# BBillot/SynthSR

Measured on AMD Instinct MI355X. Metric: training volumes/sec (160^3 fp32, 5-level U-Net), higher is better.
Workload: dtype f32; 1 GPU; configs[1]: brain_generator 160^3 batch=1 (training() defaults) + 5-level 3-D U-Net (24..384 features, Cin=2) fwd/bwd + Adam, fp32, random-init; global_batch=1, parallelism=dp1, conv_arithmetic=split

## Files before the change

synthsr_amd/csrc/conv3d.hip:

```cpp
#include "common.h"
#include <algorithm>
#include <cstddef>

SYN_DET_SETTER(conv3d)

namespace {

typedef float f32x4 __attribute__((ext_vector_type(4)));

constexpr int MAX_NT = 6;

__host__ __device__ inline int cdiv(int a, int b) { return (a + b - 1) / b; }

inline int ck_for(int Cin) { return (Cin % 24 == 0) ? 24 : 8; }
inline int ck_for_fwd(int Cin) { return (Cin % 24 == 0) ? 24 : ((Cin % 32 == 0) ? 32 : 8); }

template <int I, int N, class F>
__device__ __forceinline__ void sfor(F&& f) {
  if constexpr (I < N) {
    f(std::integral_constant<int, I>{});
    sfor<I + 1, N>(f);
  }
}
typedef unsigned int u32x4 __attribute__((ext_vector_type(4)));
// ... 54 lines not shown
      for (int c = 0; c < nx; ++c) v += w[((int64_t)((tz[a] * 3 + ty[b]) * 3 + tx[c]) * Cin_total + ci) * Cout + co];
  return v;
}

__host__ __device__ inline int64_t split_plane_floats(int NT, int ncc, int nchunks) {
  const int MT = NT <= -300 ? -300 - NT : (NT <= -200 ? -200 - NT : -100 - NT);
  return (int64_t)nchunks * ncc * (NT <= -200 ? 2 : 7) * MT * 64 * 4;
}
__device__ __forceinline__ void split_pack_pair(const float* __restrict__ w, int64_t i, int Cin_total, int ci_off, int Cin, int Cout,
                                                int mode, int ncc, int NT, int parity, int nchunks, uint32_t pc[3]) {
  const bool up = NT <= -200, fwdwin = NT <= -300;
  const int MT = fwdwin ? -300 - NT : (up ? -200 - NT : -100 - NT), nstep = up ? 2 : 7;
  uint32_t r = (uint32_t)i * 2u;
  const int j = (int)(r & 7);
  r >>= 3;
  const int lane = (int)(r & 63);
  r >>= 6;
  const int mt = (int)(r % MT);
  r /= MT;
  const int step = (int)(r % nstep);
  r /= nstep;
  const int cc = (int)(r % ncc);
  const int chunk = (int)(r / ncc);
  (void)nchunks;
  const int coe = (chunk * MT + mt) * 16 + (lane & 15);
  int tap;
  if (up) {
    const int t8 = syn_split_tap8(4 * step + (lane >> 4));
    const int pz = (parity >> 2) & 1, py = (parity >> 1) & 1, px = parity & 1;
    const int hz = (fwdwin ? pz : 1 - pz) + (t8 >> 2), hy = (fwdwin ? py : 1 - py) + ((t8 >> 1) & 1),
              hx = (fwdwin ? px : 1 - px) + (t8 & 1);
    tap = (hz * 3 + hy) * 3 + hx;
  } else {
    tap = syn_split_tap(4 * step + (lane >> 4));
  }
  float v0 = 0.f, v1 = 0.f;
  if (tap >= 0) {
    v0 = weight_value(w, tap, cc * 8 + j, coe, Cin_total, ci_off, Cin, Cout, mode, parity);
    v1 = weight_value(w, tap, cc * 8 + j + 1, coe, Cin_total, ci_off, Cin, Cout, mode, parity);
  }
  syn_split3(v0, v1, pc[0], pc[1], pc[2]);
}

__device__ __forceinline__ float stacked_pack_value(const float* __restrict__ w, int64_t idx, int Cin_total, int ci_off, int Cin,
                                                    int Cout, int mode) {
  uint32_t r = (uint32_t)idx * 2u;
  const int j = (int)(r & 7);
  r >>= 3;
  const int lane = (int)(r & 63);
  r >>= 6;
  const int tile = (int)(r % 5);
  r /= 5;
  const int step = (int)(r % 7);
  const int cc = (int)(r / 7);
  const int m = lane & 15;
  const int tap = syn_split_tap(4 * step + (lane >> 4));
  int piece, co;
  if (tile < 3) { piece = tile; co = m; }
  else if (tile == 3) { piece = m < 8 ? 0 : 1; co = 16 + (m & 7); }
  else { piece = m < 8 ? 2 : -1; co = 16 + (m & 7); }
  if (tap < 0 || piece < 0) return 0.f;
  const float v0 = weight_value(w, tap, cc * 8 + j, co, Cin_total, ci_off, Cin, Cout, mode, -1);
  const float v1 = weight_value(w, tap, cc * 8 + j + 1, co, Cin_total, ci_off, Cin, Cout, mode, -1);
  uint32_t pc[3];
  syn_split3(v0, v1, pc[0], pc[1], pc[2]);
  return __uint_as_float(pc[piece]);
}

__device__ __forceinline__ float pack_value(const float* __restrict__ w, int64_t idx, int Cin_total, int ci_off, int Cin,
                                            int Cout, int mode, int CK, int ncc, int NT, int parity, int NV,
                                            int64_t mfma_count) {
  if (NT == -400) return stacked_pack_value(w, idx, Cin_total, ci_off, Cin, Cout, mode);
  if (NT <= -100) {
    const int64_t n3 = split_plane_floats(NT, ncc, (int)mfma_count);
    uint32_t pc[3];
    split_pack_pair(w, idx % n3, Cin_total, ci_off, Cin, Cout, mode, ncc, NT, parity, (int)mfma_count, pc);
    return __uint_as_float(pc[idx / n3]);
  }
  if (NT < 0) {
    const int cin = -NT;
    const int lane = (int)(idx & 63);
    const int G = (int)(idx >> 6) * 16 + (lane >> 2);
    const int k = G / 6, g = G % 6;
    if (k >= 27 * cin) return 0.f;
    return weight_value(w, k / cin, k % cin, g * 4 + (lane & 3), Cin_total, ci_off, Cin, Cout, mode, parity);
  }
  if (NT == 0) {
    const int lane = (int)(idx & 63);
    uint32_t r = (uint32_t)(idx >> 6);
    const int rr = (int)(r % 3);
    r /= 3;
    const int qp = (int)(r % 3);
    r /= 3;
    const int tap = (int)(r % 27);
    const int cc = (int)(r / 27);
    const int G = rr * 16 + (lane >> 2);
    const int cie = cc * 24 + qp * 8 + (G / 24) * 4 + (G % 24) / 6;
    const int coe = (G % 6) * 4 + (lane & 3);
    return weight_value(w, tap, cie, coe, Cin_total, ci_off, Cin, Cout, mode, parity);
  }
  if (idx >= mfma_count) {
    uint32_t r = (uint32_t)(idx - mfma_count);
    const int v = (int)(r % NV);
    r /= NV;
    const int cil = (int)(r % CK);
    r /= CK;
    const int tap = (int)(r % 27);
    const int cc = (int)(r / 27);
    const int coutE = mode ? Cin : Cout;
    return weight_value(w, tap, cc * CK + cil, coutE - NV + v, Cin_total, ci_off, Cin, Cout, mode, parity);
  }
  const int NCG = CK / 8;
  uint32_t r = (uint32_t)idx;
  const int s = (int)(r & 1);
  r >>= 1;
  const int lane = (int)(r & 63);
  r >>= 6;
  const int nt = (int)(r % NT);
  r /= NT;
  const int cg = (int)(r % NCG);
  r /= NCG;
  const int tap = (int)(r % 27);
  r /= 27;
  const int cc = (int)(r % ncc);
  const int nc = (int)(r / ncc);
  const int kq = lane >> 4, j = lane & 15;
  const int cie = cc * CK + cg * 8 + 2 * kq + s;
  const int coe = (nc * NT + nt) * 16 + j;
  const int coutE = mode ? Cin : Cout;
  if (coe >= coutE - NV) return 0.f;
  return weight_value(w, tap, cie, coe, Cin_total, ci_off, Cin, Cout, mode, parity);
}

__global__ void pack_kernel(const float* __restrict__ w, float* __restrict__ packed, int Cin_total, int ci_off, int Cin,
                            int Cout, int mode, int CK, int ncc, int NT, int nchunks, int parity, int NV,
                            int64_t mfma_count, int64_t total) {
  if (NT <= -100 && NT != -400) {
    const int64_t n3 = total / 3;
    for (int64_t i = blockIdx.x * (int64_t)blockDim.x + threadIdx.x; i < n3; i += (int64_t)gridDim.x * blockDim.x) {
      uint32_t pc[3];
      split_pack_pair(w, i, Cin_total, ci_off, Cin, Cout, mode, ncc, NT, parity, (int)mfma_count, pc);
      packed[i] = __uint_as_float(pc[0]);
      packed[i + n3] = __uint_as_float(pc[1]);
      packed[i + 2 * n3] = __uint_as_float(pc[2]);
    }
    return;
  }
  for (int64_t idx = blockIdx.x * (int64_t)blockDim.x + threadIdx.x; idx < total;
       idx += (int64_t)gridDim.x * blockDim.x)
    packed[idx] = pack_value(w, idx, Cin_total, ci_off, Cin, Cout, mode, CK, ncc, NT, parity, NV, mfma_count);
}

constexpr int PACK_JOB_FIELDS = 14;
__global__ void pack_all_kernel(const float* __restrict__ params, float* __restrict__ packed,
                                const int64_t* __restrict__ jobs) {
  const int64_t* jb = jobs + (int64_t)blockIdx.y * PACK_JOB_FIELDS;
  const float* w = params + jb[0];
  float* dst = packed + jb[1];
  const int64_t count = jb[2];
  const int cin_total = (int)jb[3], ci_off = (int)jb[4], cin = (int)jb[5], cout = (int)jb[6], mode = (int)jb[7],
            ck = (int)jb[8], ncc = (int)jb[9], nt = (int)jb[10], parity = (int)jb[11], nv = (int)jb[12];
  const int64_t mfma_count = jb[13];
  if (nt <= -100 && nt != -400) {
    const int64_t n3 = count / 3;
    for (int64_t i = blockIdx.x * (int64_t)blockDim.x + threadIdx.x; i < n3; i += (int64_t)gridDim.x * blockDim.x) {
      uint32_t pc[3];
      split_pack_pair(w, i, cin_total, ci_off, cin, cout, mode, ncc, nt, parity, (int)mfma_count, pc);
      dst[i] = __uint_as_float(pc[0]);
      dst[i + n3] = __uint_as_float(pc[1]);
      dst[i + 2 * n3] = __uint_as_float(pc[2]);
    }
    return;
  }
  if (nt > 0 && parity >= 0 && parity < 8 && nv == 0) {
    const int64_t inner = (int64_t)(ck / 8) * nt * 128, count8 = count / 27 * 8;
    const int pz = (parity >> 2) & 1, py = (parity >> 1) & 1, px = parity & 1;
    for (int64_t i8 = blockIdx.x * (int64_t)blockDim.x + threadIdx.x; i8 < count8; i8 += (int64_t)gridDim.x * blockDim.x) {
      const int64_t q = i8 / inner, rem = i8 - q * inner;
      const int t8 = (int)(q & 7);
      const int slot = ((pz + (t8 >> 2)) * 3 + py + ((t8 >> 1) & 1)) * 3 + px + (t8 & 1);
      const int64_t idx = ((q >> 3) * 27 + (mode ? 26 - slot : slot)) * inner + rem;
      dst[idx] = pack_value(w, idx, cin_total, ci_off, cin, cout, mode, ck, ncc, nt, parity, nv, mfma_count);
    }
    return;
  }
  for (int64_t idx = blockIdx.x * (int64_t)blockDim.x + threadIdx.x; idx < count;
       idx += (int64_t)gridDim.x * blockDim.x)
    dst[idx] = pack_value(w, idx, cin_total, ci_off, cin, cout, mode, ck, ncc, nt, parity, nv, mfma_count);
}

__global__ void up_unpack_kernel(const float* __restrict__ dwc, float* __restrict__ dw, int Cin_total, int ci_off, int Cl,
                                 int Cout, int64_t total) {
  for (int64_t idx = blockIdx.x * (int64_t)blockDim.x + threadIdx.x; idx < total;
       idx += (int64_t)gridDim.x * blockDim.x) {
    const int co = (int)(idx % Cout);
    const int ci = (int)((idx / Cout) % Cl);
    const int t = (int)(idx / ((int64_t)Cout * Cl));
    const int tz = t / 9, ty = (t / 3) % 3, tx = t % 3;
    float acc = 0.f;
    for (int p = 0; p < 8; ++p) {
      const int pz = (p >> 2) & 1, py = (p >> 1) & 1, px = p & 1;
      const int sz = pz ? (tz == 2 ? 2 : 1) : (tz == 0 ? 0 : 1);
      const int sy = py ? (ty == 2 ? 2 : 1) : (ty == 0 ? 0 : 1);
      const int sx = px ? (tx == 2 ? 2 : 1) : (tx == 0 ? 0 : 1);
      acc += dwc[(((int64_t)p * 27 + (sz * 3 + sy) * 3 + sx) * Cl + ci) * Cout + co];
    }
    dw[((int64_t)t * Cin_total + ci_off + ci) * Cout + co] += acc;
  }
}
__global__ void up_clear_kernel(float* __restrict__ dwc, int Cl, int Cout, int64_t total64) {
  const int64_t inner = (int64_t)Cl * Cout;
  for (int64_t idx = blockIdx.x * (int64_t)blockDim.x + threadIdx.x; idx < total64; idx += (int64_t)gridDim.x * blockDim.x) {
    const int q = (int)(idx / inner);
    const int64_t rem = idx - (int64_t)q * inner;
    const int p = q >> 3, t8 = q & 7;
    const int slot = ((((p >> 2) & 1) + (t8 >> 2)) * 3 + ((p >> 1) & 1) + ((t8 >> 1) & 1)) * 3 + (p & 1) + (t8 & 1);
    dwc[((int64_t)p * 27 + slot) * inner + rem] = 0.f;
  }
}

template <int NT, int MT, bool RELU = false>
__device__ __forceinline__ void store_tile_rows(f32x4 (&acc)[MT][NT], float* slab, float* __restrict__ out,
                                                const float* __restrict__ bias, const float* addend, int act, int nc,
                                                int gz, int y0, int x0, int D1, int D2, int Cout, int lane) {
  const int li = lane & 15, kq = lane >> 4;
  constexpr int NW = NT * 16;
  const int c_lo = nc * NW;
  const int wc = min(Cout - c_lo, NW);
  const int wc4 = wc >> 2;
  const int nx = min(16, D2 - x0);
#pragma unroll
  for (int m = 0; m < MT; ++m) {
    const int gy = y0 + m;
    if (gy >= D1) continue;
#pragma unroll
    for (int n = 0; n < NT; ++n) {
      const int co = c_lo + n * 16 + li;
      const float bv = (bias && co < Cout) ? bias[co] : 0.f;
#pragma unroll
      for (int r = 0; r < 4; ++r) slab[(kq * 4 + r) * NW + n * 16 + li] = acc[m][n][r] + bv;
    }
    __builtin_amdgcn_wave_barrier();
    const size_t rowoff = (((size_t)gz * D1 + gy) * D2 + x0) * Cout + c_lo;
    for (int idx = lane; idx < nx * wc4; idx += 64) {
      const int x = idx / wc4, c4 = idx - x * wc4;
      float4 v = *reinterpret_cast<const float4*>(&slab[x * NW + c4 * 4]);
      const size_t o = rowoff + (size_t)x * Cout + c4 * 4;
      if (act == 2) {
        const float4 a = *reinterpret_cast<const float4*>(addend + o);
        v.x *= act_dy<RELU>(a.x);
        v.y *= act_dy<RELU>(a.y);
        v.z *= act_dy<RELU>(a.z);
        v.w *= act_dy<RELU>(a.w);
      } else if (addend) {
        const float4 a = *reinterpret_cast<const float4*>(addend + o);
        v.x += a.x;
        v.y += a.y;
        v.z += a.z;
        v.w += a.w;
      }
      if (act == 1) {
        v.x = act_f<RELU>(v.x);
        v.y = act_f<RELU>(v.y);
        v.z = act_f<RELU>(v.z);
        v.w = act_f<RELU>(v.w);
      }
      *reinterpret_cast<float4*>(out + o) = v;
    }
    __builtin_amdgcn_wave_barrier();
  }
}

constexpr int FT0 = 4, FT2 = 16;
constexpr int FH0 = 6, FH2 = 18;

struct ConvExt {
  int mode;
  const float* addend;
  int64_t wstride;
  int64_t valu_off;
};

__host__ __device__ inline uint32_t up_tapmask(int p, bool flipped) {
  uint32_t m = 0;
  for (int sz = 0; sz < 3; ++sz)
    for (int sy = 0; sy < 3; ++sy)
      for (int sx = 0; sx < 3; ++sx) {
        const int pz = (p >> 2) & 1, py = (p >> 1) & 1, px = p & 1;
        const bool ok = (pz ? sz >= 1 : sz <= 1) && (py ? sy >= 1 : sy <= 1) && (px ? sx >= 1 : sx <= 1);
        if (ok) {
          const int t = flipped ? (((2 - sz) * 3 + (2 - sy)) * 3 + (2 - sx)) : ((sz * 3 + sy) * 3 + sx);
          m |= 1u << t;
        }
      }
  return m;
}

template <int CK, int NT, int MT, bool KSPLIT, int NV, bool RELU = false>
__global__ __launch_bounds__(256, 2) void conv3d_fwd_kernel(const float* __restrict__ in, const float* __restrict__ wp,
                                                            const float* __restrict__ bias, float* __restrict__ out,
                                                            int D0, int D1, int D2, int Cin, int Cout, int ncc,
                                                            int tiles1, int tiles2, int act, ConvExt ext) {
  extern __shared__ __attribute__((aligned(16))) float lds[];
  constexpr int FT1 = MT, FH1 = MT + 2, FHV = FH0 * FH1 * FH2;
  constexpr int CKP = CK + 4;
  constexpr int NCG = CK / 8;
  constexpr int C4 = CK / 4;
  const int dbg = act >> 8;
  act &= 0xff;
  const int tid = threadIdx.x, lane = tid & 63, wave = tid >> 6;
  int t;
  {
    const int nwg = gridDim.x, b = blockIdx.x;
    const int q = nwg >> 3, r = nwg & 7, xcd = b & 7, j = b >> 3;
    t = (xcd < r ? xcd * (q + 1) : r * (q + 1) + (xcd - r) * q) + j;
  }
  const int t2 = t % tiles2;
  t /= tiles2;
  const int t1 = t % tiles1;
  const int t0 = t / tiles1;
  const int z0 = t0 * FT0, y0 = t1 * FT1, x0 = t2 * FT2;
  const int nc = blockIdx.y;

  f32x4 acc[MT][NT];
#pragma unroll
  for (int m = 0; m < MT; ++m)
#pragma unroll
    for (int n = 0; n < NT; ++n) acc[m][n] = (f32x4){0.f, 0.f, 0.f, 0.f};

  static_assert(NV == 0 || (MT == 4 && !KSPLIT && CK == 24), "VALU share needs the 4x4x16 tile");
  float accv[NV > 0 ? NV : 1];
#pragma unroll
  for (int v = 0; v < (NV > 0 ? NV : 1); ++v) accv[v] = 0.f;
  const int vbase = ((wave * FH1 + (lane >> 4)) * FH2 + (lane & 15)) * CKP;

  const int li = lane & 15, kq = lane >> 4;
  int a_base[MT];
#pragma unroll
  for (int m = 0; m < MT; ++m) a_base[m] = ((wave * FH1 + m) * FH2 + li) * CKP + 2 * kq;

  const float* wl = wp + (size_t)nc * ncc * 27 * NCG * NT * 128 + lane * 2;
// ... 3024 lines not shown
                       tiles2, ntiles);
  else
    hipLaunchKernelGGL(conv3d_wgrad_c2_kernel<1>, dim3(gx), dim3(256), 0, st, in, dout, partial, s[0], s[1], s[2], tiles1,
                       tiles2, ntiles);
  if (hipGetLastError() != hipSuccess) return SYNTHSR_ELAUNCH;
  const int nrow = 27 * Cin;
  hipLaunchKernelGGL(rows_reduce_kernel, dim3(cdiv((nrow + 1) * 24, 64), 32), dim3(64), 0, st, partial, gx, dw, dbias, nrow,
                     Cin, ext.cin_total, ext.ci_off);
  return hipGetLastError() == hipSuccess ? SYNTHSR_OK : SYNTHSR_ELAUNCH;
}

template <int NTAPS>
int dispatch_wgrad(const float* in, const float* dout, float* dw, const int shape[3], int Cin, int Cout, hipStream_t st,
                   const WgExt& ext) {
  if constexpr (NTAPS == 8) {
    if (up_wgrad_takes_split(shape, Cin, Cout)) {
      const int rc = syn_split_upwgrad(in, dout, dw, shape, Cin, Cout, cfg().nprod, st);
      if (rc != SYNTHSR_EINVAL) return rc;
    }
    const int64_t vox = (int64_t)shape[0] * shape[1] * shape[2];
    const int tiles0 = cdiv(shape[0], FT0), tiles1 = cdiv(shape[1], 4), tiles2 = cdiv(shape[2], FT2);
    const int ntiles = tiles0 * tiles1 * tiles2, ncc = Cin / 24;
    if (Cout == 24 && (Cin % 24) == 0 && PLAN_P4 && ntiles >= 768 && vox * Cin * 4 < (1ll << 31) &&
        vox * 8 * Cout * 4 < (1ll << 31) && !(PLAN_DBG & 16)) {
      const size_t smem = (size_t)FH0 * 6 * FH2 * 28 * sizeof(float);
      static SynOncePerDevice attr_done;
      if (auto once_ = attr_done.first()) {
        (void)hipFuncSetAttribute(reinterpret_cast<const void*>(conv3d_up_wgrad_p4_kernel),
                                  hipFuncAttributeMaxDynamicSharedMemorySize, (int)smem);
      }
      int gx = std::max(8, ((512 / (ncc * 2)) / 8) * 8);
      while (gx > 8 && gx > ntiles) gx -= 8;
      DetRun det;
      float* no_dbias = nullptr;
      if (const int rc_ = syn_det_prepare(&det, &dw, &no_dbias, 8 * ext.dwstride, Cout, gx, st)) return rc_;
      hipLaunchKernelGGL(conv3d_up_wgrad_p4_kernel, dim3(gx, ncc * 2), dim3(256), smem, st, in, dout, dw, shape[0], shape[1],
                         shape[2], Cin, tiles1, tiles2, ntiles, ext.dwstride, ext.dbg, det.stride);
      if (hipGetLastError() != hipSuccess) return SYNTHSR_ELAUNCH;
      return syn_det_finish(&det, st);
    }
  }
  if constexpr (NTAPS == 27) {
    if (Cin <= 2 && Cout == 24 && PLAN_P4 && (int64_t)shape[0] * shape[1] * shape[2] * Cout * 4 < (1ll << 31))
      return launch_wgrad_c2(in, dout, dw, ext.dbias, shape, Cin, st, ext);
    if (wgrad_takes_split(shape, Cin, Cout)) {
      const int rc = syn_split_wgrad(in, dout, dw, ext.dbias, shape, ext.cin_total, ext.ci_off, Cin, Cout, cfg().nprod, st);
      if (rc != SYNTHSR_EINVAL) return rc;
    }
  }
  if constexpr (NTAPS == 27) {
    const int64_t vox = (int64_t)shape[0] * shape[1] * shape[2];
    if (Cout == 24 && (Cin % 24) == 0 && PLAN_P4 && vox * Cin * 4 < (1ll << 31) && vox * Cout * 4 < (1ll << 31) &&
        !(PLAN_DBG & 16)) {
      const int tiles0 = cdiv(shape[0], FT0), tiles1 = cdiv(shape[1], 4), tiles2 = cdiv(shape[2], FT2);
      const int ntiles = tiles0 * tiles1 * tiles2, ncc = Cin / 24;
      const size_t smem = (size_t)FH0 * 6 * FH2 * 28 * sizeof(float);
      static SynOncePerDevice attr_done;
      if (auto once_ = attr_done.first()) {
        (void)hipFuncSetAttribute(reinterpret_cast<const void*>(conv3d_wgrad_p4_kernel),
                                  hipFuncAttributeMaxDynamicSharedMemorySize, (int)smem);
      }
      int gx = std::max(8, ((512 / ncc) / 8) * 8);
      while (gx > 8 && gx > ntiles) gx -= 8;
      DetRun det;
      float* dbias = ext.dbias;
      if (const int rc_ = syn_det_prepare(&det, &dw, &dbias, (int64_t)27 * ext.cin_total * Cout, Cout, gx, st)) return rc_;
      hipLaunchKernelGGL(conv3d_wgrad_p4_kernel, dim3(gx, ncc), dim3(256), smem, st, in, dout, dw, shape[0], shape[1],
                         shape[2], Cin, tiles1, tiles2, ntiles, ext.cin_total, ext.ci_off, ext.dbg, dbias, det.stride);
      if (hipGetLastError() != hipSuccess) return SYNTHSR_ELAUNCH;
      return syn_det_finish(&det, st);
    }
  }
  const int CK = ck_for(Cin);
  const int nt_all = cdiv(Cout, 16);
  const int nco = cdiv(nt_all, 3);
  const int NT = cdiv(nt_all, nco);
  if (CK == 24) {
    if (NT == 1) return launch_wgrad<24, 1, 1, NTAPS>(in, dout, dw, shape, Cin, Cout, st, ext);
    if (NT == 2) return launch_wgrad<24, 2, 1, NTAPS>(in, dout, dw, shape, Cin, Cout, st, ext);
    if constexpr (NTAPS == 27) return launch_wgrad<24, 3, 2, 27>(in, dout, dw, shape, Cin, Cout, st, ext);
    return launch_wgrad<24, 3, 1, NTAPS>(in, dout, dw, shape, Cin, Cout, st, ext);
  }
  if (NT == 1) return launch_wgrad<8, 1, 1, NTAPS>(in, dout, dw, shape, Cin, Cout, st, ext);
  if (NT == 2) return launch_wgrad<8, 2, 1, NTAPS>(in, dout, dw, shape, Cin, Cout, st, ext);
  return launch_wgrad<8, 3, 1, NTAPS>(in, dout, dw, shape, Cin, Cout, st, ext);
}

}

extern "C" {

int64_t synthsr_conv3d_pack_ex(const synthsr_conv_ctx* ctx, const float* w, float* packed, const int shape[3], int Cin_total,
                               int ci_off, int Cin, int Cout, int mode, int up, synthsr_stream_t stream) {
  const CtxScope scope(ctx);
  if (!scope.ok) return SYNTHSR_EINVAL;
  if (!shape || Cin < 1 || Cout < 1 || ci_off < 0 || ci_off + Cin > Cin_total || (mode != 0 && mode != 1) ||
      shape[0] < 1 || shape[1] < 1 || shape[2] < 1 || up < 0 || up > 2)
    return SYNTHSR_EINVAL;
  const int CinE = mode ? Cout : Cin, CoutE = mode ? Cin : Cout;
  const int kind = !up ? 1 : ((up == 1) == (mode == 0) ? 2 : 0);
  const FwdPlan pl = plan_fwd(shape, CinE, CoutE, kind);
  const int64_t per = pl.count();
  if (per >= (1ll << 31)) return SYNTHSR_EINVAL;
  const int64_t total = per * (up ? 8 : 1);
  if (!packed) return total;
  if (!w) return SYNTHSR_EINVAL;
  for (int p = 0; p < (up ? 8 : 1); ++p) {
    hipLaunchKernelGGL(pack_kernel, dim3(syn_grid(per, 256)), dim3(256), 0, (hipStream_t)stream, w, packed + p * per,
                       Cin_total, ci_off, Cin, Cout, mode, pl.ck, pl.ncc, pl.pack_nt(), pl.nchunks,
                       up ? p + (up == 2 ? 8 : 0) : -1, pl.nv, pl.mfma_count(), per);
    if (hipGetLastError() != hipSuccess) return SYNTHSR_ELAUNCH;
  }
  return total;
}

int64_t synthsr_conv3d_pack(const synthsr_conv_ctx* ctx, const float* w, float* packed, const int shape[3], int Cin, int Cout,
                            int mode, synthsr_stream_t stream) {
  return synthsr_conv3d_pack_ex(ctx, w, packed, shape, Cin, 0, Cin, Cout, mode, 0, stream);
}

int synthsr_conv3d_plan(const synthsr_conv_ctx* ctx, const int shape[3], int CinE, int CoutE, int plain, int64_t out[8]) {
  const CtxScope scope(ctx);
  if (!scope.ok) return SYNTHSR_EINVAL;
  if (!shape || !out || CinE < 1 || CoutE < 1 || shape[0] < 1 || shape[1] < 1 || shape[2] < 1) return SYNTHSR_EINVAL;
  const FwdPlan pl = plan_fwd(shape, CinE, CoutE, plain);
  out[0] = pl.ck;
  out[1] = pl.ncc;
  out[2] = pl.pack_nt();
  out[3] = pl.nchunks;
  out[4] = pl.mt;
  out[5] = (pl.split == 1 && syn_split_fwd_halves(shape, CinE, pl.nchunks, pl.stacked, cfg().nprod)) ? 2 : pl.ksplit;
  out[6] = pl.nv;
  out[7] = pl.count();
  return SYNTHSR_OK;
}

int synthsr_conv3d_wgrad_runs_split(const synthsr_conv_ctx* ctx, const int shape[3], int Cin, int Cout) {
  const CtxScope scope(ctx);
  if (!scope.ok) return SYNTHSR_EINVAL;
  if (!shape || Cin < 1 || Cout < 1 || shape[0] < 1 || shape[1] < 1 || shape[2] < 1) return SYNTHSR_EINVAL;
  return (Cin > 2 || Cout != 24) && wgrad_takes_split(shape, Cin, Cout) ? 1 : 0;
}

int synthsr_conv3d_up_wgrad_runs_split(const synthsr_conv_ctx* ctx, const int lo_shape[3], int Cl, int Cout) {
  const CtxScope scope(ctx);
  if (!scope.ok) return SYNTHSR_EINVAL;
  if (!lo_shape || Cl < 1 || Cout < 1 || lo_shape[0] < 1 || lo_shape[1] < 1 || lo_shape[2] < 1) return SYNTHSR_EINVAL;
  return up_wgrad_takes_split(lo_shape, Cl, Cout) ? 1 : 0;
}

int synthsr_conv3d_pack_all(const float* params, float* packed, const int64_t* jobs_dev, int njobs,
                            synthsr_stream_t stream) {
  if (!params || !packed || !jobs_dev || njobs < 1) return SYNTHSR_EINVAL;
  hipLaunchKernelGGL(pack_all_kernel, dim3(256, njobs), dim3(256), 0, (hipStream_t)stream, params, packed, jobs_dev);
  return hipGetLastError() == hipSuccess ? SYNTHSR_OK : SYNTHSR_ELAUNCH;
}

__global__ void stride_unpack_kernel(const float* __restrict__ dwc, float* __restrict__ dw, int Ci, int Co, int64_t total) {
  for (int64_t idx = blockIdx.x * (int64_t)blockDim.x + threadIdx.x; idx < total; idx += (int64_t)gridDim.x * blockDim.x) {
    const int co = (int)(idx % Co);
    const int ci = (int)((idx / Co) % Ci);
    const int t = (int)(idx / ((int64_t)Co * Ci));
    const int tz = t / 9, ty = (t / 3) % 3, tx = t % 3;
    const int p = ((tz & 1) << 2) | ((ty & 1) << 1) | (tx & 1);
    const int slot = ((1 - (tz >> 1)) * 3 + (1 - (ty >> 1))) * 3 + (1 - (tx >> 1));
    dw[idx] += dwc[(((int64_t)p * 27 + slot) * Co + co) * Ci + ci];
  }
}

int synthsr_conv3d_stride_unpack(const float* dwc, float* dw, int Ci, int Co, synthsr_stream_t stream) {
  if (!dwc || !dw || Ci < 1 || Co < 1) return SYNTHSR_EINVAL;
  const int64_t total = (int64_t)27 * Ci * Co;
  hipLaunchKernelGGL(stride_unpack_kernel, dim3(syn_grid(total, 256)), dim3(256), 0, (hipStream_t)stream, dwc, dw, Ci, Co,
                     total);
  return hipGetLastError() == hipSuccess ? SYNTHSR_OK : SYNTHSR_ELAUNCH;
}

int synthsr_conv3d_up_unpack(float* dwc, float* dw, int Cin_total, int ci_off, int Cl, int Cout, synthsr_stream_t stream) {
  if (!dwc || !dw || Cl < 1 || Cout < 1 || ci_off < 0 || ci_off + Cl > Cin_total) return SYNTHSR_EINVAL;
  const int64_t total = (int64_t)27 * Cl * Cout;
  hipLaunchKernelGGL(up_unpack_kernel, dim3(syn_grid(total, 256)), dim3(256), 0, (hipStream_t)stream, dwc, dw, Cin_total,
                     ci_off, Cl, Cout, total);
  if (hipGetLastError() != hipSuccess) return SYNTHSR_ELAUNCH;
  const int64_t total64 = (int64_t)64 * Cl * Cout;
  hipLaunchKernelGGL(up_clear_kernel, dim3(syn_grid(total64, 256)), dim3(256), 0, (hipStream_t)stream, dwc, Cl, Cout, total64);
  return hipGetLastError() == hipSuccess ? SYNTHSR_OK : SYNTHSR_ELAUNCH;
}

int synthsr_conv3d_fwd(const synthsr_conv_ctx* ctx, const float* in, const float* wpacked, const float* bias, float* out,
                       const int shape[3], int Cin, int Cout, int act, synthsr_stream_t stream) {
  const CtxScope scope(ctx);
  if (!scope.ok) return SYNTHSR_EINVAL;
  if (!in || !wpacked || !out || !shape || Cin < 1 || Cout < 1 || shape[0] < 1 || shape[1] < 1 || shape[2] < 1 ||
      (act != 0 && act != 1 && act != 3))
    return SYNTHSR_EINVAL;
  const FwdPlan pl = plan_fwd(shape, Cin, Cout);
  if (pl.split)
    return syn_split_fwd(in, wpacked, bias, nullptr, out, shape, Cin, Cout, pl.mt, pl.nchunks, act, nullptr, nullptr, 0,
                         pl.stacked, cfg().nprod, (hipStream_t)stream);
  const ConvExt ext{0, nullptr, 0, pl.mfma_count()};
  if (pl.ck == 24) return dispatch_fwd<24>(in, wpacked, bias, out, shape, Cin, Cout, pl, act, (hipStream_t)stream, ext);
  if (pl.ck == 32) return dispatch_fwd<32>(in, wpacked, bias, out, shape, Cin, Cout, pl, act, (hipStream_t)stream, ext);
  return dispatch_fwd<8>(in, wpacked, bias, out, shape, Cin, Cout, pl, act, (hipStream_t)stream, ext);
}

int synthsr_conv3d_fwd_add(const synthsr_conv_ctx* ctx, const float* in, const float* wpacked, const float* bias,
                           const float* addend, float* out, const int shape[3], int Cin, int Cout, int act,
                           synthsr_stream_t stream) {
  const CtxScope scope(ctx);
  if (!scope.ok) return SYNTHSR_EINVAL;
  if (!in || !wpacked || !out || !shape || Cin < 1 || Cout < 1 || shape[0] < 1 || shape[1] < 1 || shape[2] < 1 ||
      act < 0 || act > 4 || ((act == 2 || act == 4) && (!addend || addend == out)))
    return SYNTHSR_EINVAL;
  const FwdPlan pl = plan_fwd(shape, Cin, Cout);
  if (pl.split)
    return syn_split_fwd(in, wpacked, bias, addend, out, shape, Cin, Cout, pl.mt, pl.nchunks, act, nullptr, nullptr, 0,
                         pl.stacked, cfg().nprod, (hipStream_t)stream);
  const ConvExt ext{0, addend, 0, pl.mfma_count()};
  if (pl.ck == 24) return dispatch_fwd<24>(in, wpacked, bias, out, shape, Cin, Cout, pl, act, (hipStream_t)stream, ext);
  if (pl.ck == 32) return dispatch_fwd<32>(in, wpacked, bias, out, shape, Cin, Cout, pl, act, (hipStream_t)stream, ext);
  return dispatch_fwd<8>(in, wpacked, bias, out, shape, Cin, Cout, pl, act, (hipStream_t)stream, ext);
}

int synthsr_conv3d_fwd_stats(const synthsr_conv_ctx* ctx, const float* in, const float* wpacked, const float* bias, float* out,
                             const int shape[3], int Cin, int Cout, int act, float* stats, double* ws, synthsr_stream_t stream) {
  const CtxScope scope(ctx);
  if (!scope.ok) return SYNTHSR_EINVAL;
  if (!in || !wpacked || !out || !shape || !stats || !ws || Cin < 1 || Cout < 1 || shape[0] < 1 || shape[1] < 1 ||
      shape[2] < 1 || (act != 0 && act != 1 && act != 3))
    return SYNTHSR_EINVAL;
  const int64_t nvox = (int64_t)shape[0] * shape[1] * shape[2];
  const FwdPlan pl = plan_fwd(shape, Cin, Cout);
  if (pl.split) {
    float* partial = ctx_scratch((size_t)512 * 2 * Cout * sizeof(float));
    if (!partial) return SYNTHSR_EWORKSPACE;
    return syn_split_fwd(in, wpacked, bias, nullptr, out, shape, Cin, Cout, pl.mt, pl.nchunks, act, stats, partial, 0,
                         pl.stacked, cfg().nprod, (hipStream_t)stream);
  }
  if (pl.p4 && nvox * Cin * 4 < (1ll << 31))
    return launch_fwd_p4(in, wpacked, bias, out, shape, Cin, pl, act, (hipStream_t)stream, nullptr, stats);
  const int rc = synthsr_conv3d_fwd(ctx, in, wpacked, bias, out, shape, Cin, Cout, act, stream);
  if (rc != SYNTHSR_OK) return rc;
  return synthsr_bn_stats(out, nvox, Cout, stats, ws, stream);
}

int synthsr_conv3d_up_fwd(const synthsr_conv_ctx* ctx, const float* lo, const float* wpacked8, const float* bias,
                          const float* addend, float* out, const int lo_shape[3], int Cl, int Cout, int act,
                          synthsr_stream_t stream) {
  const CtxScope scope(ctx);
  if (!scope.ok) return SYNTHSR_EINVAL;
  if (!lo || !wpacked8 || !out || !lo_shape || Cl < 1 || Cout < 1 || lo_shape[0] < 1 || lo_shape[1] < 1 ||
      lo_shape[2] < 1 || (act != 0 && act != 1 && act != 3))
    return SYNTHSR_EINVAL;
  const FwdPlan pl = plan_fwd(lo_shape, Cl, Cout, 2);
  if (pl.split)
    return syn_split_upfwd(lo, wpacked8, bias, addend, out, lo_shape, Cl, Cout, pl.mt, act, cfg().nprod, (hipStream_t)stream);
  const int64_t wstride = pl.count();
  const ConvExt ext{1, addend, wstride, pl.mfma_count()};
  if (pl.ck == 24) return dispatch_fwd<24>(lo, wpacked8, bias, out, lo_shape, Cl, Cout, pl, act, (hipStream_t)stream, ext);
  if (pl.ck == 32) return dispatch_fwd<32>(lo, wpacked8, bias, out, lo_shape, Cl, Cout, pl, act, (hipStream_t)stream, ext);
  return dispatch_fwd<8>(lo, wpacked8, bias, out, lo_shape, Cl, Cout, pl, act, (hipStream_t)stream, ext);
}

int synthsr_conv3d_up_dgrad(const synthsr_conv_ctx* ctx, const float* dout, const float* wpacked8, float* dlo,
                            const int lo_shape[3], int Cl, int Cout, synthsr_stream_t stream) {
  const CtxScope scope(ctx);
  if (!scope.ok) return SYNTHSR_EINVAL;
  if (!dout || !wpacked8 || !dlo || !lo_shape || Cl < 1 || Cout < 1 || lo_shape[0] < 1 || lo_shape[1] < 1 ||
      lo_shape[2] < 1)
    return SYNTHSR_EINVAL;
  const FwdPlan pl = plan_fwd(lo_shape, Cout, Cl, 0);
  if (pl.split)
    return syn_split_fwd(dout, wpacked8, nullptr, nullptr, dlo, lo_shape, Cout, Cl, pl.mt, pl.nchunks, 0, nullptr, nullptr, 2, 0,
                         cfg().nprod, (hipStream_t)stream);
  const int64_t wstride = pl.count();
  const ConvExt ext{2, nullptr, wstride, pl.mfma_count()};
  if (pl.ck == 24) return dispatch_fwd<24>(dout, wpacked8, nullptr, dlo, lo_shape, Cout, Cl, pl, 0, (hipStream_t)stream, ext);
  if (pl.ck == 32) return dispatch_fwd<32>(dout, wpacked8, nullptr, dlo, lo_shape, Cout, Cl, pl, 0, (hipStream_t)stream, ext);
  return dispatch_fwd<8>(dout, wpacked8, nullptr, dlo, lo_shape, Cout, Cl, pl, 0, (hipStream_t)stream, ext);
}


extern "C" __attribute__((visibility("hidden"))) int syn_det_enabled() { return det_on(); }
extern "C" __attribute__((visibility("hidden"))) int syn_det_prepare(DetRun* d, float** dw, float** dbias, int64_t dw_elems,
                                                                      int cout, int gx, hipStream_t st) {
  return det_prepare_impl(d, dw, dbias, dw_elems, cout, gx, st);
}
extern "C" __attribute__((visibility("hidden"))) int syn_det_finish(const DetRun* d, hipStream_t st) {
  return det_finish_impl(d, st);
}
extern "C" int syn_det_set_pointwise(SynDet*);
extern "C" int syn_det_set_critic(SynDet*);
extern "C" int syn_det_set_ssim(SynDet*);
extern "C" int syn_det_set_conv_bf16(SynDet*);
constexpr long long DET_SCRATCH_FLOATS = 16ll << 20;

int synthsr_set_deterministic(int on) {
  if (hipDeviceSynchronize() != hipSuccess) return SYNTHSR_ELAUNCH;
  int cur = -1;
  if (hipGetDevice(&cur) != hipSuccess || cur < 0 || cur >= SYN_MAX_DEVICES) return SYNTHSR_EINVAL;
  SynDeviceState& ds = g_dev[cur];
  if (on && !ds.det_state) {
    SynDet* state = nullptr;
    float* scratch = nullptr;
    if (hipMalloc(reinterpret_cast<void**>(&state), sizeof(SynDet)) != hipSuccess) return SYNTHSR_ELAUNCH;
    bool ok = hipMalloc(reinterpret_cast<void**>(&scratch), DET_SCRATCH_FLOATS * sizeof(float)) == hipSuccess;
    if (ok) {
      SynDet* h = new SynDet();
// ... 80 lines not shown
```

Measured before the change: 53.85 volumes/s.

## Load-balance weight packing across jobs with prefix-sum chunking and vectorized stores

The weight-pack kernel used to launch a 2-D grid of 256 blocks per job, so small jobs wasted blocks and large ones were under-parallelised. It now builds an in-shared-memory prefix sum of per-job chunk counts and has a fixed 2048-block grid stride over global chunks. Each thread also produces four packed values per iteration and writes them as a 16-byte store when the destination is aligned. This adds a per-block prefix scan and more index arithmetic, and it can issue several launches when there are very many jobs.

Result: no change. 53.57 volumes/s (-0.5%).

```diff
diff --git a/synthsr_amd/csrc/conv3d.hip b/synthsr_amd/csrc/conv3d.hip
--- a/synthsr_amd/csrc/conv3d.hip
+++ b/synthsr_amd/csrc/conv3d.hip
@@ -230,41 +230,197 @@
 }
 
 constexpr int PACK_JOB_FIELDS = 14;
-__global__ void pack_all_kernel(const float* __restrict__ params, float* __restrict__ packed,
-                                const int64_t* __restrict__ jobs) {
-  const int64_t* jb = jobs + (int64_t)blockIdx.y * PACK_JOB_FIELDS;
-  const float* w = params + jb[0];
-  float* dst = packed + jb[1];
+constexpr int PACK_ALL_GRID = 2048;
+constexpr int PACK_ALL_MAX_JOBS = 16384;
+
+__device__ __forceinline__ bool pack_job_is_split(int nt) { return nt <= -100 && nt != -400; }
+__device__ __forceinline__ bool pack_job_is_window(int nt, int parity, int nv) {
+  return nt > 0 && parity >= 0 && parity < 8 && nv == 0;
+}
+__device__ __forceinline__ int64_t pack_job_units(const int64_t* __restrict__ jb) {
   const int64_t count = jb[2];
-  const int cin_total = (int)jb[3], ci_off = (int)jb[4], cin = (int)jb[5], cout = (int)jb[6], mode = (int)jb[7],
-            ck = (int)jb[8], ncc = (int)jb[9], nt = (int)jb[10], parity = (int)jb[11], nv = (int)jb[12];
-  const int64_t mfma_count = jb[13];
-  if (nt <= -100 && nt != -400) {
-    const int64_t n3 = count / 3;
-    for (int64_t i = blockIdx.x * (int64_t)blockDim.x + threadIdx.x; i < n3; i += (int64_t)gridDim.x * blockDim.x) {
-      uint32_t pc[3];
-      split_pack_pair(w, i, cin_total, ci_off, cin, cout, mode, ncc, nt, parity, (int)mfma_count, pc);
-      dst[i] = __uint_as_float(pc[0]);
-      dst[i + n3] = __uint_as_float(pc[1]);
-      dst[i + 2 * n3] = __uint_as_float(pc[2]);
+  const int nt = (int)jb[10];
+  if (pack_job_is_split(nt)) return count / 12;
+  if (pack_job_is_window(nt, (int)jb[11], (int)jb[12])) return count / 27 * 2;
+  return (count + 3) / 4;
+}
+__device__ __forceinline__ int pack_job_chunk_units(int nt) { return pack_job_is_split(nt) ? 256 : 512; }
+
+__device__ __forceinline__ void split_pack_quad(const float* __restrict__ w, uint32_t i, int Cin_total, int ci_off, int Cin, int Cout,
+                                                int mode, int ncc, int NT, int parity, uint32_t pc[3][4]) {
+  const bool up = NT <= -200, fwdwin = NT <= -300;
+  const int MT = fwdwin ? -300 - NT : (up ? -200 - NT : -100 - NT), nstep = up ? 2 : 7;
+  uint32_t r = i >> 2;
+  const int lane = (int)(r & 63);
+  r >>= 6;
+  const int mt = (int)(r % MT);
+  r /= MT;
+  const int step = (int)(r % nstep);
+  r /= nstep;
+  const int cc = (int)(r % ncc);
+  const int chunk = (int)(r / ncc);
+  const int coe = (chunk * MT + mt) * 16 + (lane & 15);
+  int tap;
+  if (up) {
+    const int t8 = syn_split_tap8(4 * step + (lane >> 4));
+    const int pz = (parity >> 2) & 1, py = (parity >> 1) & 1, px = parity & 1;
+    const int hz = (fwdwin ? pz : 1 - pz) + (t8 >> 2), hy = (fwdwin ? py : 1 - py) + ((t8 >> 1) & 1),
+              hx = (fwdwin ? px : 1 - px) + (t8 & 1);
+    tap = (hz * 3 + hy) * 3 + hx;
+  } else {
+    tap = syn_split_tap(4 * step + (lane >> 4));
+  }
+#pragma unroll
+  for (int p = 0; p < 4; ++p) {
+    float v0 = 0.f, v1 = 0.f;
+    if (tap >= 0) {
+      v0 = weight_value(w, tap, cc * 8 + 2 * p, coe, Cin_total, ci_off, Cin, Cout, mode, parity);
+      v1 = weight_value(w, tap, cc * 8 + 2 * p + 1, coe, Cin_total, ci_off, Cin, Cout, mode, parity);
+    }
+    syn_split3(v0, v1, pc[0][p], pc[1][p], pc[2][p]);
+  }
+}
+
+__device__ __forceinline__ void pack_value4(const float* __restrict__ w, int64_t idx, int64_t count, int Cin_total, int ci_off,
+                                            int Cin, int Cout, int mode, int CK, int ncc, int NT, int parity, int NV,
+                                            int64_t mfma_count, float v[4]) {
+  if (NT == -400) {
+    uint32_t r = (uint32_t)idx >> 2;
+    const int lane = (int)(r & 63);
+    r >>= 6;
+    const int tile = (int)(r % 5);
+    r /= 5;
+    const int step = (int)(r % 7);
+    const int cc = (int)(r / 7);
+    const int m = lane & 15;
+    const int tap = syn_split_tap(4 * step + (lane >> 4));
+    int piece, co;
+    if (tile < 3) { piece = tile; co = m; }
+    else if (tile == 3) { piece = m < 8 ? 0 : 1; co = 16 + (m & 7); }
+    else { piece = m < 8 ? 2 : -1; co = 16 + (m & 7); }
+#pragma unroll
+    for (int p = 0; p < 4; ++p) {
+      v[p] = 0.f;
+      if (tap >= 0 && piece >= 0) {
+        const float v0 = weight_value(w, tap, cc * 8 + 2 * p, co, Cin_total, ci_off, Cin, Cout, mode, -1);
+        const float v1 = weight_value(w, tap, cc * 8 + 2 * p + 1, co, Cin_total, ci_off, Cin, Cout, mode, -1);
+        uint32_t pc[3];
+        syn_split3(v0, v1, pc[0], pc[1], pc[2]);
+        v[p] = __uint_as_float(pc[piece]);
+      }
     }
     return;
   }
-  if (nt > 0 && parity >= 0 && parity < 8 && nv == 0) {
-    const int64_t inner = (int64_t)(ck / 8) * nt * 128, count8 = count / 27 * 8;
+  if (NT > 0 && idx + 3 < mfma_count) {
+    const int NCG = CK / 8;
+    uint32_t r = (uint32_t)idx >> 1;
+    const int lane = (int)(r & 63);
+    r >>= 6;
+    const int nt = (int)(r % NT);
+    r /= NT;
+    const int cg = (int)(r % NCG);
+    r /= NCG;
+    const int tap = (int)(r % 27);
+    r /= 27;
+    const int cc = (int)(r % ncc);
+    const int nc = (int)(r / ncc);
+    const int coutE = mode ? Cin : Cout;
+#pragma unroll
+    for (int e = 0; e < 4; ++e) {
+      const int cie = cc * CK + cg * 8 + 2 * (lane >> 4) + (e & 1);
+      const int coe = (nc * NT + nt) * 16 + (lane & 15) + (e >> 1);
+      v[e] = coe >= coutE - NV ? 0.f : weight_value(w, tap, cie, coe, Cin_total, ci_off, Cin, Cout, mode, parity);
+    }
+    return;
+  }
+#pragma unroll
+  for (int e = 0; e < 4; ++e)
+    if (idx + e < count) v[e] = pack_value(w, idx + e, Cin_total, ci_off, Cin, Cout, mode, CK, ncc, NT, parity, NV, mfma_count);
+}
+
+__global__ __launch_bounds__(256) void pack_all_kernel(const float* __restrict__ params, float* __restrict__ packed,
+                                                       const int64_t* __restrict__ jobs, int njobs) {
+  extern __shared__ int pack_pre[];
+  for (int j = threadIdx.x; j < njobs; j += blockDim.x) {
+    const int64_t* jb = jobs + (int64_t)j * PACK_JOB_FIELDS;
+    const int cu = pack_job_chunk_units((int)jb[10]);
+    pack_pre[j + 1] = (int)((pack_job_units(jb) + cu - 1) / cu);
+  }
+  if (threadIdx.x == 0) pack_pre[0] = 0;
+  __syncthreads();
+  if (threadIdx.x < 64) {
+    int carry = 0;
+    for (int j0 = 0; j0 < njobs; j0 += 64) {
+      const int j = j0 + (int)threadIdx.x;
+      int x = j < njobs ? pack_pre[j + 1] : 0;
+#pragma unroll
+      for (int o = 1; o < 64; o <<= 1) {
+        const int y = __shfl_up(x, o, 64);
+        if ((int)threadIdx.x >= o) x += y;
+      }
+      if (j < njobs) pack_pre[j + 1] = x + carry;
+      carry += __shfl(x, 63, 64);
+    }
+  }
+  __syncthreads();
+  const int nchunks = pack_pre[njobs];
+  const bool base16 = (reinterpret_cast<uintptr_t>(packed) & 15) == 0;
+  int job = 0;
+  for (int c = blockIdx.x; c < nchunks; c += gridDim.x) {
+    while (pack_pre[job + 1] <= c) ++job;
+    job = __builtin_amdgcn_readfirstlane(job);
+    const int64_t* jb = jobs + (int64_t)job * PACK_JOB_FIELDS;
+    const float* w = params + jb[0];
+    float* dst = packed + jb[1];
+    const int64_t count = jb[2];
+    const int cin_total = (int)jb[3], ci_off = (int)jb[4], cin = (int)jb[5], cout = (int)jb[6], mode = (int)jb[7],
+              ck = (int)jb[8], ncc = (int)jb[9], nt = (int)jb[10], parity = (int)jb[11], nv = (int)jb[12];
+    const int64_t mfma_count = jb[13];
+    const bool vec = base16 && (jb[1] & 3) == 0;
+    const int64_t units = pack_job_units(jb);
+    const int cu = pack_job_chunk_units(nt);
+    const int64_t u0 = (int64_t)(c - pack_pre[job]) * cu;
+    const int64_t u1 = min(u0 + cu, units);
+    if (pack_job_is_split(nt)) {
+      const int64_t n3 = count / 3;
+      for (int64_t u = u0 + threadIdx.x; u < u1; u += blockDim.x) {
+        uint32_t pc[3][4];
+        split_pack_quad(w, (uint32_t)u * 4u, cin_total, ci_off, cin, cout, mode, ncc, nt, parity, pc);
+#pragma unroll
+        for (int q = 0; q < 3; ++q) {
+          float* d = dst + q * n3 + u * 4;
+          if (vec && (n3 & 3) == 0) {
+            *reinterpret_cast<u32x4*>(d) = (u32x4){pc[q][0], pc[q][1], pc[q][2], pc[q][3]};
+          } else {
+#pragma unroll
+            for (int e = 0; e < 4; ++e) d[e] = __uint_as_float(pc[q][e]);
+          }
+        }
+      }
+      continue;
+    }
+    const bool window = pack_job_is_window(nt, parity, nv);
+    const uint32_t inner = (uint32_t)(ck / 8) * (uint32_t)max(nt, 0) * 128u;
     const int pz = (parity >> 2) & 1, py = (parity >> 1) & 1, px = parity & 1;
-    for (int64_t i8 = blockIdx.x * (int64_t)blockDim.x + threadIdx.x; i8 < count8; i8 += (int64_t)gridDim.x * blockDim.x) {
-      const int64_t q = i8 / inner, rem = i8 - q * inner;
-      const int t8 = (int)(q & 7);
-      const int slot = ((pz + (t8 >> 2)) * 3 + py + ((t8 >> 1) & 1)) * 3 + px + (t8 & 1);
-      const int64_t idx = ((q >> 3) * 27 + (mode ? 26 - slot : slot)) * inner + rem;
-      dst[idx] = pack_value(w, idx, cin_total, ci_off, cin, cout, mode, ck, ncc, nt, parity, nv, mfma_count);
-    }
-    return;
-  }
-  for (int64_t idx = blockIdx.x * (int64_t)blockDim.x + threadIdx.x; idx < count;
-       idx += (int64_t)gridDim.x * blockDim.x)
-    dst[idx] = pack_value(w, idx, cin_total, ci_off, cin, cout, mode, ck, ncc, nt, parity, nv, mfma_count);
+    for (int64_t u = u0 + threadIdx.x; u < u1; u += blockDim.x) {
+      int64_t idx = u * 4;
+      if (window) {
+        const uint32_t i8 = (uint32_t)idx, q = i8 / inner, rem = i8 - q * inner;
+        const int t8 = (int)(q & 7);
+        const int slot = ((pz + (t8 >> 2)) * 3 + py + ((t8 >> 1) & 1)) * 3 + px + (t8 & 1);
+        idx = ((int64_t)(q >> 3) * 27 + (mode ? 26 - slot : slot)) * inner + rem;
+      }
+      float v[4];
+      pack_value4(w, idx, count, cin_total, ci_off, cin, cout, mode, ck, ncc, nt, parity, nv, mfma_count, v);
+      if (vec && idx + 3 < count) {
+        *reinterpret_cast<float4*>(dst + idx) = make_float4(v[0], v[1], v[2], v[3]);
+      } else {
+#pragma unroll
+        for (int e = 0; e < 4; ++e)
+          if (idx + e < count) dst[idx + e] = v[e];
+      }
+    }
+  }
 }
 
 __global__ void up_unpack_kernel(const float* __restrict__ dwc, float* __restrict__ dw, int Cin_total, int ci_off, int Cl,
@@ -3595,8 +3751,13 @@
 int synthsr_conv3d_pack_all(const float* params, float* packed, const int64_t* jobs_dev, int njobs,
                             synthsr_stream_t stream) {
   if (!params || !packed || !jobs_dev || njobs < 1) return SYNTHSR_EINVAL;
-  hipLaunchKernelGGL(pack_all_kernel, dim3(256, njobs), dim3(256), 0, (hipStream_t)stream, params, packed, jobs_dev);
-  return hipGetLastError() == hipSuccess ? SYNTHSR_OK : SYNTHSR_ELAUNCH;
+  for (int j0 = 0; j0 < njobs; j0 += PACK_ALL_MAX_JOBS) {
+    const int n = std::min(njobs - j0, PACK_ALL_MAX_JOBS);
+    hipLaunchKernelGGL(pack_all_kernel, dim3(PACK_ALL_GRID), dim3(256), (n + 1) * sizeof(int), (hipStream_t)stream, params, packed,
+                       jobs_dev + (int64_t)j0 * PACK_JOB_FIELDS, n);
+    if (hipGetLastError() != hipSuccess) return SYNTHSR_ELAUNCH;
+  }
+  return SYNTHSR_OK;
 }
 
 __global__ void stride_unpack_kernel(const float* __restrict__ dwc, float* __restrict__ dw, int Ci, int Co, int64_t total) {
```
